# unirestore/UniRestore

Hardware: AMD Instinct MI355X
Metric: restored 512x512 images/sec @ 20 denoise steps (whole job) (higher is better)
Workload: dtype bf16; 1 GPU; PIR 512x512 batch=8/GPU, 20 DDIM steps, bf16, hipGraph replay (BASELINE.json configs[1]; configs[2] shape for N=8); global_batch=8, per_gpu_batch=8, image=512, denoise_steps=20, parallelism=image-parallel dp1, weights=seeded random init (no checkpoints reachable)

## Files before the change

### unirestore_amd/csrc/igemm.hip

```cpp
#include "igemm_impl.h"

namespace urk {
#define UR_DECLARE(name)                                                                                             \
  ConvLaunch name##_bf16(void* k, size_t ws_bytes);                                                                 \
  ConvLaunch name##_f16(void* k, size_t ws_bytes);                                                                  \
  static ConvLaunch name(ConvK& k, size_t ws_bytes) { return (k.f16 ? name##_f16 : name##_bf16)(&k, ws_bytes); }
UR_CONV_LAUNCHERS(UR_DECLARE)
#undef UR_DECLARE
}

namespace {

ConvLaunch dispatch_conv(ConvK& k, bool pair, size_t ws_bytes) {
  if (k.KH == 3 && k.stride == 1 && k.pad_t == 1 && k.pad_l == 1 && k.kcm && k.staged_ok_ && !pair && k.nbatch == 1 &&
      k.OW % 32 == 0 && k.OH % 8 == 0 && k.OH == (k.ups ? 2 * k.H : k.H) && k.OW == (k.ups ? 2 * k.W : k.W) && !k.yt) {
    const bool ok128 = k.Cout % 128 == 0, ok160 = k.Cout % 160 == 0;
    const long long tm8 = (long long)k.N * (k.OH / 8) * (k.OW / 32);
    auto eff = [](long long t) { return t <= 128 ? (double)(t * (256 / t)) / 256.0 : (double)t / (double)(((t + 255) / 256) * 256); };
    const bool use160 = ok160 && (!ok128 || eff(tm8 * (k.Cout / 160)) >= eff(tm8 * (k.Cout / 128)));
    const long long tiles8 = tm8 * (use160 ? k.Cout / 160 : k.Cout / 128);
    if ((ok128 || ok160) && tiles8 >= 64) {
      if (use160) return urk::halo_8x32_160(k, ws_bytes);
      return urk::halo_8x32_128(k, ws_bytes);
    }
  }
  if (k.KH == 3 && k.stride == 1 && k.pad_t == 1 && k.pad_l == 1 && k.kcm && !pair && k.nbatch == 1 && !k.ups && k.C2 == 0 &&
      k.Cout <= 32 && k.OW % 32 == 0 && k.OH % 8 == 0 && k.OH == k.H && k.OW == k.W && !k.yt && !k.gn_part && !k.gn_ab && !k.row_stats && !k.ln_stats &&
      !k.bias_img && (long long)k.N * (k.OH / 8) * (k.OW / 32) >= 128)
    return urk::halo_thin_32(k, ws_bytes);
  const bool himg_ups = k.ups && k.OH == 16 && k.OW == 16 && k.H == 8 && k.W == 8;
  if (k.KH == 3 && k.stride == 1 && k.pad_t == 1 && k.pad_l == 1 && k.kcm && k.staged_ok_ && !pair && k.nbatch == 1 &&
      ((!k.ups && k.OH == k.H && k.OW == k.W) || himg_ups) && !k.yt && k.Cout % 128 == 0 && k.nk >= 36) {
    if (k.wf && k.OH == 8 && k.OW == 8 && k.N <= 16 && k.Cin % 256 == 0 && k.nk >= 72 && k.y && k.ws && !k.gn_ab && !k.row_stats && !k.ln_stats &&
        (long long)(k.nk / 36) * k.M * k.Cout * 4 <= (long long)ws_bytes)
      return urk::wstream_8x8(k, ws_bytes);
    if (k.OH == 16 && k.OW == 16) return urk::himg_16x16(k, ws_bytes);
    if (k.OH == 8 && k.OW == 8 && k.N % 4 == 0) {
      return urk::himg_8x8x4(k, ws_bytes);
    }
  }
  if (k.KH == 1 && k.stride == 1 && !k.ups && k.C2 == 0 && k.staged_ok_ && k.Cout % 256 == 0 && !k.yt && (k.act == UR_ACT_GEGLU || k.act == UR_ACT_GATE) &&
      (long long)((k.M + 255) / 256) * (k.Cout / 256) * k.nbatch >= 200 && (long long)k.M * k.ldx < (1ll << 31) - 256)
  {
    auto fill = [](long long t) { return (double)t / (double)(((t + 255) / 256) * 256); };
    const long long tm = (k.M + 255) / 256;
    if (k.Cout % 320 == 0 && k.nbatch == 1 && !k.bias_img && fill(tm * (k.Cout / 320)) > fill(tm * (k.Cout / 256)))
      return urk::gemm_256x320_pair(k, ws_bytes);
    return urk::gemm_256x256(k, ws_bytes);
  }
  const bool use_v1 = k.KH == 1 && k.nk <= 10;
  const long long blocks128 = (long long)((k.M + 127) / 128) * ((k.Cout + 127) / 128) * k.nbatch;
  const bool g1 = k.KH == 1 && k.stride == 1 && !k.ups && k.C2 == 0 && k.pad_t == 0 && k.pad_l == 0 && k.OH == k.H && k.OW == k.W &&
                  (long long)k.M * k.ldx + k.Ktot < (1ll << 31) - 256;
  auto nosplit = [&](int bm, int bn) { return (long long)((k.M + bm - 1) / bm) * ((k.Cout + bn - 1) / bn) * k.nbatch >= 200 || k.nk < 8 || !k.ws; };
  if (k.KH == 1 && !pair && k.Cout > 64) {
    const long long blocks64 = (long long)((k.M + 63) / 64) * ((k.Cout + 63) / 64) * k.nbatch;
    if (blocks128 < 200 && g1 && blocks64 >= 128 && blocks64 <= 256 && k.nk >= 8 && k.nk <= 48) return urk::g1_64x64_deep(k, ws_bytes);
    if (g1 && blocks128 < 200 && k.nk > 24 && k.nk <= 96 && (long long)((k.M + 127) / 128) * ((k.Cout + 63) / 64) * k.nbatch >= 256)
      return urk::g1_128x64_deep(k, ws_bytes);
    if (blocks128 < 200 && g1 && ((blocks64 >= 128 && k.nk <= 24) || (blocks64 >= 256 && k.nk <= 48))) return urk::g1_64x64(k, ws_bytes);
    if (blocks128 < 200 && k.nk <= 24) return g1 && nosplit(64, 64) ? urk::g1_64x64(k, ws_bytes) : urk::v1_64x64(k, ws_bytes);
    if (use_v1 && blocks128 > 256 && blocks128 < 400 && k.Cout % 128 == 0) return g1 && nosplit(128, 64) ? urk::g1_128x64(k, ws_bytes) : urk::v1_128x64(k, ws_bytes);
  }
  if (use_v1) {
    if (pair) return urk::v1_128x128(k, ws_bytes);
    if (k.Cout <= 32) return urk::v1_256x32(k, ws_bytes);
    if (k.Cout <= 64) return urk::v1_128x64(k, ws_bytes);
    if (k.Cout % 160 == 0 && k.Cout % 128 != 0) return g1 && nosplit(128, 160) ? urk::g1_128x160(k, ws_bytes) : urk::v1_128x160(k, ws_bytes);
    return g1 && nosplit(128, 128) ? urk::g1_128x128(k, ws_bytes) : urk::v1_128x128(k, ws_bytes);
  }
  if (k.Cout <= 32) return urk::v2_256x32(k, ws_bytes);
  if (k.Cout <= 64 && !pair) return urk::v2_128x64(k, ws_bytes);
  const bool n160 = !pair && k.Cout % 160 == 0 && k.Cout % 128 != 0;
  const long long big_tiles = (long long)((k.M + 255) / 256) * ((k.Cout + (n160 ? 159 : 127)) / (n160 ? 160 : 128)) * k.nbatch;
  if (g1 && !pair && big_tiles < 256) {
    const long long t160 = k.Cout % 160 == 0 ? (long long)((k.M + 127) / 128) * (k.Cout / 160) : 0;
    const long long t128 = (long long)((k.M + 127) / 128) * ((k.Cout + 127) / 128);
    auto fill = [](long long t) { return t <= 0 ? 0.0 : (double)t / (double)(((t + 255) / 256) * 256); };
    if (t160 >= 200 && fill(t160) >= fill(t128)) return urk::g1_128x160(k, ws_bytes);
    if (t128 >= 200) return urk::g1_128x128(k, ws_bytes);
  }
  if (big_tiles >= 160) {
    if (n160 && g1) return urk::g1_128x160(k, ws_bytes);
    if (n160) return urk::v2_256x160(k, ws_bytes);
    return urk::v2_256x128(k, ws_bytes);
  }
  if (k.Cout % 160 == 0 && k.Cout % 128 != 0 && !pair) return urk::v1_128x160(k, ws_bytes);
  return urk::v1_128x128(k, ws_bytes);
}

}

static int conv_impl(const ur_conv_desc* d, ur_stream_t stream, ur_conv_plan* plan, ur_conv_launch_info* info = nullptr) {
  UR_REQUIRE(d && d->x && d->w, "null x/w");
  UR_REQUIRE(d->KH == d->KW && (d->KH == 1 || d->KH == 3), "only 1x1 and 3x3 kernels");
  UR_REQUIRE(d->C1 > 0 && d->C1 % 8 == 0 && d->C2 % 8 == 0 && d->ldx % 8 == 0, "Cin/ldx must be multiples of 8");
  UR_REQUIRE(d->C2 == 0 || (d->x2 && d->ldx2 % 8 == 0), "virtual concat needs x2");
  UR_REQUIRE(d->Cout > 0 && d->Cout % 4 == 0 && d->ldw % 8 == 0, "Cout%4, ldw%8");
  UR_REQUIRE(d->nbatch >= 1 && d->stride >= 1 && d->OH > 0 && d->OW > 0, "bad dims");
  UR_REQUIRE(d->y || d->yt || d->gn_part, "no output requested");
  UR_REQUIRE_DT(d->dtype);
  const bool pair = d->act == UR_ACT_GEGLU || d->act == UR_ACT_GATE;
  if (pair && d->Cout % 64 != 0)
    return ur::fail(UR_E_UNSUPPORTED, "ur_conv2d_nhwc: pair activations (GEGLU / SimpleGate) need Cout % 64 == 0 (32-row a|g interleave)");
  UR_REQUIRE(!d->y || (d->out_f32 ? d->ldy % 4 == 0 : d->ldy % 4 == 0), "ldy%4");
  UR_REQUIRE(!d->residual || d->ldr % 4 == 0, "ldr%4");
  UR_REQUIRE(!d->yt || (d->t_rows > 0 && d->n_split % 4 == 0 && !pair), "bad transposed-output spec");

  ConvK k;
  k.x = (const uint16_t*)d->x; k.x2 = (const uint16_t*)d->x2; k.w = (const uint16_t*)d->w; k.bias = d->bias;
  k.res = (const uint16_t*)d->residual; k.y = d->y; k.yt = (uint16_t*)d->yt;
  k.ws = d->workspace;
  k.N = d->N; k.H = d->H; k.W = d->W; k.C1 = d->C1; k.ldx = d->ldx; k.C2 = d->C2; k.ldx2 = d->ldx2;
  k.Cin = d->C1 + d->C2; k.Cout = d->Cout; k.ldw = d->ldw; k.ldy = d->ldy; k.ldr = d->ldr;
  k.KH = d->KH; k.KW = d->KW; k.stride = d->stride; k.pad_t = d->pad_t; k.pad_l = d->pad_l;
  k.OH = d->OH; k.OW = d->OW; k.OHW = d->OH * d->OW; k.ups = d->upsample2x; k.act = d->act; k.out_f32 = d->out_f32;
  k.n_split = d->yt ? d->n_split : d->Cout; k.t_rows = d->t_rows; k.t_ld = d->t_ld;
  k.out_scale = d->out_scale;
  k.M = d->N * d->OH * d->OW; k.Ktot = d->KH * d->KW * k.Cin; k.nk = (k.Ktot + 63) / 64; k.nbatch = d->nbatch;
  k.bs_x = d->bs_x; k.bs_x2 = d->bs_x2; k.bs_w = d->bs_w; k.bs_bias = d->bs_bias; k.bs_y = d->bs_y; k.bs_r = d->bs_r; k.bias_img = d->bias_img_stride;
  UR_REQUIRE(k.M > 0, "empty problem");
  UR_REQUIRE((long long)d->N * d->H * d->W * (long long)std::max(d->ldx, d->ldx2) < (1ll << 31) &&
                 (long long)d->Cout * d->ldw < (1ll << 31), "tensor too large for 32-bit element offsets");

  k.kcm = d->k_chunk_major; k.wf = (const uint16_t*)d->w_frag; k.wmajor = 0; k.xgm = 0; k.xbn = 0; k.patch_tw = 0;
  UR_REQUIRE(!k.kcm || (k.Cin % 64 == 0 && d->C1 % 64 == 0), "k_chunk_major needs C1 and C1+C2 to be multiples of 64");
  k.gn_part = d->gn_part; k.gn_ab = d->gn_ab; k.gn_silu = d->gn_silu; k.f16 = d->dtype == UR_DT_F16; k.gn_fused = 0; k.gn_parts = 0;
  k.ln_parts = d->ln_parts;
  k.row_stats = d->row_stats; k.ln_stats = d->ln_stats; k.ln_colsum = d->ln_colsum; k.ln_eps = d->ln_eps; k.ln_dim = d->ln_dim;
  UR_REQUIRE(!d->ln_stats || (d->ln_colsum && d->ln_dim > 0), "ln_stats needs ln_colsum / ln_dim");
  UR_REQUIRE(!(d->bias_img_stride && (pair || d->ln_stats || d->yt)), "per-image bias rows do not combine with pair activations / LayerNorm folding / transposed columns");
  k.staged_ok_ = (d->y ? (!d->out_f32 && ((d->ldy | d->bs_y) & 7) == 0) : d->gn_part != nullptr) &&
                 (!d->residual || ((d->ldr | d->bs_r) & 7) == 0);
  UR_REQUIRE(!d->gn_part || (!d->out_f32 && !d->yt), "gn_part needs a plain 16-bit output (or none)");
  hipStream_t s = (hipStream_t)stream;
  const double flops = 2.0 * k.M * (double)k.Cout * k.Ktot * k.nbatch;
  const double bytes = 2.0 * ((double)k.M * k.Cin + (double)k.Cout * k.Ktot + (double)k.M * k.Cout) * k.nbatch;
  const char* fam = d->KH == 3 ? "conv3x3_igemm" : "gemm1x1_igemm";
  static const bool prof_shapes = getenv("UR_PROF_SHAPES") != nullptr;
  if (prof_shapes) {
    static std::map<std::string, int> interned;
    char buf[128];
    snprintf(buf, sizeof buf, "%s M%d N%d K%d s%d u%d b%d a%d", d->KH == 3 ? "c3" : "g1", k.M, k.Cout, k.Ktot, d->stride, d->upsample2x,
             k.nbatch, d->act);
    fam = interned.emplace(buf, 0).first->first.c_str();
  }
  const ConvLaunch launch = dispatch_conv(k, pair, d->workspace_bytes);
  const bool group_loop = k.nbatch > 1 && d->KH == 3 && k.kcm && k.stride == 1 && !pair && !k.gn_part && !k.row_stats && !k.ln_stats &&
                          !k.yt && !k.gn_ab && !k.out_f32 && k.staged_ok_ && k.Cout % 128 == 0 && !k.bias_img && k.C2 == 0;
  auto group_k = [&](int b) {
    ConvK kb = k;
    kb.nbatch = 1;
    kb.x = k.x + b * k.bs_x; kb.w = k.w + b * k.bs_w; kb.bias = k.bias ? k.bias + b * k.bs_bias : nullptr;
    kb.res = k.res ? k.res + b * k.bs_r : nullptr;
    kb.y = reinterpret_cast<uint16_t*>(k.y) + b * k.bs_y;
    kb.bs_x = kb.bs_w = kb.bs_bias = kb.bs_y = kb.bs_r = 0;
    return kb;
  };
  if (plan) {
    plan->row_stat_parts = d->row_stats ? (k.splitk > 1 ? 1 : k.tiles_n) : 0;
    plan->gn_parts = k.gn_parts; plan->gn_fused = k.gn_fused; plan->prologue_ok = launch.prologue_ok;
  }
  if (info) {
    ConvK kb = group_loop ? group_k(0) : k;
    const ConvLaunch l = group_loop ? dispatch_conv(kb, pair, d->workspace_bytes) : launch;
    info->launcher = l.id; info->splitk = kb.splitk; info->nk_per_split = kb.nk_per_split;
    const ReducePlan r = kb.splitk > 1 ? plan_splitk_reduce(kb) : ReducePlan{-1, 0};
    info->reduce = r.kind; info->reduce_ri = r.ri;
    info->gn_pass = k.gn_part && !k.gn_fused && !group_loop;
    info->group_loop = group_loop;
  }
  if (plan || info) return UR_OK;
  if (!d->y && d->gn_part && (!k.gn_fused || k.splitk > 1))
    return ur::fail(UR_E_UNSUPPORTED, "ur_conv2d_nhwc: y == NULL needs a launch whose epilogue writes gn_part (see ur_conv2d_plan)");
// ... 70 lines not shown
```

### unirestore_amd/csrc/igemm_impl.h

```cpp
#pragma once
#include <cstdio>
#include <cstdlib>
#include <map>
#include <string>

#include "common.h"

static __device__ uint4 g_zero_page[8];
typedef uint32_t ig_u32x4 __attribute__((ext_vector_type(4)));

struct ConvLaunch {
  int (*launch)(void* k, hipStream_t s);
  int prologue_ok;
  int id;
};

namespace {

struct ConvK {
  const uint16_t* x; const uint16_t* x2; const uint16_t* w; const float* bias; const uint16_t* res;
  void* y; uint16_t* yt; float* ws; float* gn_part; const float* gn_ab;
  float* row_stats; const float* ln_stats; const float* ln_colsum; float ln_eps; int ln_dim, ln_parts;
  int N, H, W, C1, ldx, C2, ldx2, Cin, Cout, ldw, ldy, ldr, KH, KW, stride, pad_t, pad_l, OH, OW, OHW;
  int ups, act, out_f32, n_split, t_rows, t_ld;
// ... 1594 lines not shown
    unsigned wvo[WPIECES];
#pragma unroll
    for (int q = 0; q < WPIECES; ++q) {
      const int row = n0 + q * 8 + lr;
      wvo[q] = row < p.Cout ? (unsigned)row * (unsigned)p.ldw * 2u + ((q & 1) ? ck1 : ck0) : IG_OOB;
    }
    int hpx[HNEED];
    auto dma_w = [&](int kt, int ring, int q0, int q1) {
      const unsigned so = (unsigned)(kt0 + min(kt, nk - 1)) * 128u;
#pragma unroll
      for (int q = q0; q < q1; ++q) ig_lds_dma16(wring_lds + ring * WBYTES + q * 1024, wvo[q], rs_w, so);
    };
    auto dma_h = [&](int c, int h) {
      const int cb = (c_begin + min(c, nchunk - 1)) * 64;
      const bool second = cb >= p.C1;
      const unsigned ld2 = (unsigned)(second ? p.ldx2 : p.ldx) * 2u;
      const unsigned so = (unsigned)(second ? cb - p.C1 : cb) * 2u;
#pragma unroll
      for (int j = 0; j < HPER; ++j) {
        const int q = h * HPER + j;
        if (h < 16 && q < HNEED) {
          const unsigned vo = hpx[q] >= 0 ? (unsigned)hpx[q] * ld2 + ((q & 1) ? ck1 : ck0) : IG_OOB;
          const unsigned m0v = hbuf_lds + (c & 1) * HBYTES + q * 1024;
          if (second) ig_lds_dma16(m0v, vo, rs_x2, so);
          else ig_lds_dma16(m0v, vo, rs_x1, so);
        }
      }
    };
    auto halo_count = [](int h) -> int { return (h >= 16 || h * HPER >= HNEED) ? 0 : (HNEED - h * HPER < HPER ? HNEED - h * HPER : HPER); };
    auto dma_ab = [&](int c) {
      const unsigned vo = lane < 32 ? (unsigned)((img * 2 + (lane >> 4 & 1)) * p.Cin + (lane & 15) * 4) * 4u : IG_OOB;
      ig_lds_dma16(abuf_lds + (c & 1) * 1024, vo, rs_ab, (unsigned)((c_begin + min(c, nchunk - 1)) * 64) * 4u);
    };
    if (gnp && do_h) dma_ab(0);
    if (do_w) dma_w(1, 1, 0, WPIECES);
    if (do_h) {
#pragma unroll
      for (int q = 0; q < HNEED; ++q) hpx[q] = halo_pixel(q * 8 + lr);
    }
    if (gnp && do_h) {
      if (do_w) asm volatile("s_waitcnt vmcnt(%0)" ::"n"(WPIECES) : "memory");
      else asm volatile("s_waitcnt vmcnt(0)" ::: "memory");
    }
    __builtin_amdgcn_s_barrier();
    if (gnp) __builtin_amdgcn_s_barrier();
    for (int c = 0; c < nchunk; ++c) {
#pragma unroll
      for (int tap = 0; tap < 9; ++tap) {
        const int kt = c * 9 + tap;
        if (do_w) dma_w(kt + 2, (tap + 2) % 3, 0, WH);
        if (do_h) {
          dma_h(c + 1, 2 * tap);
          if (gnp && tap == 0) dma_ab(c + 1);
        }
        if (kt + 1 == nk) asm volatile("s_waitcnt vmcnt(0)" ::: "memory");
        else if (do_w && do_h) asm volatile("s_waitcnt vmcnt(%0)" ::"n"(WH + halo_count(2 * tap) + ((gnp && tap == 0) ? 1 : 0)) : "memory");
        else if (do_w) asm volatile("s_waitcnt vmcnt(%0)" ::"n"(WH) : "memory");
        else asm volatile("s_waitcnt vmcnt(%0)" ::"n"(halo_count(2 * tap) + ((gnp && tap == 0) ? 1 : 0)) : "memory");
        __builtin_amdgcn_s_barrier();
        if (kt + 1 < nk) {
          if (do_w) dma_w(kt + 2, (tap + 2) % 3, WH, WPIECES);
          if (do_h) dma_h(c + 1, 2 * tap + 1);
        }
        __builtin_amdgcn_s_barrier();
      }
    }
    return;
  }

  const int wm = wid % WM, wn = wid / WM;
  const int chunk = ps ^ ((((wid & 1) << 2) + (lr >> 1)) & 7);
  static_assert(HTAP % 2 == 0, "piece parity");
  int hpix[8];
#pragma unroll
  for (int t = 0; t < 8; ++t) hpix[t] = (wid < HTAP && t * HTAP + wid < HNEED) ? halo_pixel((t * HTAP + wid) * 8 + lr) : -1;
  {
    const ig_u32x4 rs_w = ig_make_rsrc(p.w, (unsigned long long)p.Cout * p.ldw * 2);
    const int cb = c_begin * 64;
    const bool second = cb >= p.C1;
    const ig_u32x4 rs_x = second ? ig_make_rsrc(p.x2, (unsigned long long)p.N * p.H * p.W * p.ldx2 * 2) : ig_make_rsrc(p.x, (unsigned long long)p.N * p.H * p.W * p.ldx * 2);
    const unsigned ld2 = (unsigned)(second ? p.ldx2 : p.ldx) * 2u, so = (unsigned)(second ? cb - p.C1 : cb) * 2u;
    if (wid_s < HTAP) {
#pragma unroll
      for (int t = 0; t < 8; ++t)
        if (t * HTAP + wid_s < HNEED)
          ig_lds_dma16(hbuf_lds + (t * HTAP + wid_s) * 1024, hpix[t] >= 0 ? (unsigned)hpix[t] * ld2 + chunk * 16u : IG_OOB, rs_x, so);
    }
#pragma unroll
    for (int j = 0; j < (WPIECES + NW - 1) / NW; ++j) {
      const int q = wid_s + NW * j;
      if (q < WPIECES) {
        const int row = n0 + q * 8 + lr;
        ig_lds_dma16(wring_lds + q * 1024, row < p.Cout ? (unsigned)row * (unsigned)p.ldw * 2u + chunk * 16u : IG_OOB, rs_w, (unsigned)kt0 * 128u);
      }
    }
  }
  auto gn_slot = [&](int c, int t) {
    if (hpix[t] >= 0)
      gn_piece_inplace<F16>(hbuf + (c & 1) * HBYTES + (t * HTAP + wid) * 1024 + lane * 16, gn_load_ab(abuf + (c & 1) * 1024, chunk), p.gn_silu != 0);
  };
  f32x16 acc[FN][FM];
#pragma unroll
  for (int a = 0; a < FN; ++a)
#pragma unroll
    for (int b = 0; b < FM; ++b)
#pragma unroll
      for (int e = 0; e < 16; ++e) acc[a][b][e] = 0.f;
  const int frow = lane & 31, fhalf = lane >> 5;
  const unsigned aw_lds = wring_lds + (wn * WTN + frow) * 128 + ((fhalf ^ ((frow >> 1) & 7)) << 4);
  static_assert(((WTN >> 1) & 7) == 0, "the wave's weight rows must keep the swizzle phase of fragment row 0");
  auto tap_addr = [&](int cc, int tp, unsigned (&ab)[FM]) -> unsigned {
    const int dy = tp / 3, dx = tp % 3;
#pragma unroll
    for (int b = 0; b < FM; ++b) {
      const int hrow = (wm * FM + b + dy) * PW + dx + frow;
      ab[b] = hbuf_lds + (cc & 1) * HBYTES + hrow * 128 + ((fhalf ^ ((hrow >> 1) & 7)) << 4);
    }
    return aw_lds + (tp % 3) * WBYTES;
  };
  KPipeRings<FM, FN> rings;
  kpipe_init(rings);
  asm volatile("s_waitcnt vmcnt(0)" ::: "memory");
  __builtin_amdgcn_s_barrier();
  if (gnp) {
#pragma unroll
    for (int t = 0; t < 8; ++t) gn_slot(0, t);
    asm volatile("s_waitcnt lgkmcnt(0)" ::: "memory");
    __builtin_amdgcn_s_barrier();
  }
  {
    unsigned ab0[FM];
    const unsigned aw0 = tap_addr(0, 0, ab0);
    kpipe<FM, FN, F16, 0>(acc, rings, ab0, aw0, ab0, aw0);
  }
  for (int c = 0; c < nchunk; ++c) {
    const bool next_chunk = c + 1 < nchunk;
#pragma unroll
    for (int tap = 0; tap < 9; ++tap) {
      if (gnp && tap >= 2 && next_chunk) gn_slot(c + 1, tap >= 2 ? tap - 2 : 0);
      if (gnp && tap == 0 && c > 0) gn_slot(c, 7);
      unsigned ab[FM], abn[FM];
      const unsigned aw = tap_addr(c, tap, ab), awn = tap_addr(c + (tap == 8 ? 1 : 0), (tap + 1) % 9, abn);
      kpipe<FM, FN, F16, 1>(acc, rings, ab, aw, abn, awn);
      __builtin_amdgcn_s_barrier();
      kpipe<FM, FN, F16, 2>(acc, rings, ab, aw, abn, awn);
      __builtin_amdgcn_s_barrier();
    }
  }
  kpipe_drain(rings);
  asm volatile("s_nop 15\n\ts_nop 7" ::: "memory");
  igemm_epilogue<FM, FN, WTM, WTN, BM, BN, NT, F16, false>(p, acc, m0, n0, wm, wn, lane, 0, sz, smem);
}

template <int TH, int BN, int WM, int WN>
struct HaloThin {
  static constexpr int NW = WM * WN, HPIX = (TH + 2) * 34, HSLOTS = (HPIX + 8 * NW - 1) / (8 * NW);
  static constexpr int HBYTES = HSLOTS * NW * 1024;
  static constexpr int lds = 2 * HBYTES + 3 * (BN * 128 > NW * 1024 ? BN * 128 : NW * 1024) + 2048;
  static_assert(lds <= 160 * 1024, "LDS budget");
  static int plan(ConvK& k, size_t) {
    k.tiles_m = k.N * (k.OH / TH) * (k.OW / 32);
    k.tiles_n = (k.Cout + BN - 1) / BN;
    k.splitk = 1;
    k.nk_per_split = k.nk;
    set_gn_plan(k, false, 0);
    return 0;
  }
  static int launch(ConvK& k, hipStream_t s) {
    k.patch_tw = 32;
    static ur::DeviceOnce attr_once;
    if (auto once_guard = attr_once.first()) {
      hipFuncSetAttribute(reinterpret_cast<const void*>(&igemm_halo_kernel<TH, BN, WM, WN, UR_TU_F16 != 0, false>), hipFuncAttributeMaxDynamicSharedMemorySize, lds);
    }
    UR_F16_SWITCH(k, hipLaunchKernelGGL((igemm_halo_kernel<TH, BN, WM, WN, F16, false>), dim3(k.tiles_m * k.tiles_n, 1), dim3(NW * 64), lds, s, k));
    return ur::check_launch("ur_conv2d_nhwc");
  }
};

template <int TH, int BN, int WM, int WN>
struct Halo {
  static constexpr int NW = WM * WN, BM = TH * 32, HPIX = (TH + 2) * 34, HSLOTS = (HPIX + 8 * NW - 1) / (8 * NW);
  static constexpr int HBYTES = HSLOTS * NW * 1024;
  static constexpr int lds_loop = 2 * HBYTES + 3 * BN * 128 + 2048, lds_epi = epi_lds_bytes<BM, BN, NW * 64>();
  static constexpr int lds = lds_loop > lds_epi ? lds_loop : lds_epi;
  static_assert(lds <= 160 * 1024, "LDS budget");
  static constexpr bool GN_OK = BN <= 128;
  static int plan(ConvK& k, size_t ws_bytes) {
    k.tiles_m = k.N * (k.OH / TH) * (k.OW / 32);
    k.tiles_n = (k.Cout + BN - 1) / BN;
    const int nchunk = k.nk / 9;
    const long long tiles = (long long)k.tiles_m * k.tiles_n;
    plan_splitk(k, ws_bytes, tiles <= 128 && k.ws && k.y ? std::min<long long>(256 / tiles, std::max(1, nchunk / 2)) : 1, 9);
    set_gn_plan(k, true, (k.OH / TH) * (k.OW / 32));
    return GN_OK;
  }
  static int launch(ConvK& k, hipStream_t s) {
    k.patch_tw = 32;
    static ur::DeviceOnce attr_once;
    if (auto once_guard = attr_once.first()) {
      hipFuncSetAttribute(reinterpret_cast<const void*>(&igemm_halo_kernel<TH, BN, WM, WN, UR_TU_F16 != 0, false>), hipFuncAttributeMaxDynamicSharedMemorySize, lds);
      hipFuncSetAttribute(reinterpret_cast<const void*>(&igemm_halo_kernel<TH, BN, WM, WN, UR_TU_F16 != 0, GN_OK>), hipFuncAttributeMaxDynamicSharedMemorySize, lds);
      hipFuncSetAttribute(reinterpret_cast<const void*>(&igemm_halo_ws_kernel<TH, BN, WM, WN, UR_TU_F16 != 0, false>), hipFuncAttributeMaxDynamicSharedMemorySize, lds);
      hipFuncSetAttribute(reinterpret_cast<const void*>(&igemm_halo_ws_kernel<TH, BN, WM, WN, UR_TU_F16 != 0, GN_OK>), hipFuncAttributeMaxDynamicSharedMemorySize, lds);
    }
    static const bool no_ws = getenv("UR_HALO_NOWS") != nullptr;
    if (no_ws) {
      if (GN_OK && k.gn_ab) UR_F16_SWITCH(k, hipLaunchKernelGGL((igemm_halo_kernel<TH, BN, WM, WN, F16, GN_OK>), dim3(k.tiles_m * k.tiles_n, k.splitk), dim3(NW * 64), lds, s, k));
      else UR_F16_SWITCH(k, hipLaunchKernelGGL((igemm_halo_kernel<TH, BN, WM, WN, F16, false>), dim3(k.tiles_m * k.tiles_n, k.splitk), dim3(NW * 64), lds, s, k));
    } else {
      static const bool ld1 = getenv("UR_HALO_LD1") != nullptr;
      const dim3 blk((NW + (ld1 ? 1 : 2)) * 64);
      if (GN_OK && k.gn_ab) UR_F16_SWITCH(k, hipLaunchKernelGGL((igemm_halo_ws_kernel<TH, BN, WM, WN, F16, GN_OK>), dim3(k.tiles_m * k.tiles_n, k.splitk), blk, lds, s, k));
      else UR_F16_SWITCH(k, hipLaunchKernelGGL((igemm_halo_ws_kernel<TH, BN, WM, WN, F16, false>), dim3(k.tiles_m * k.tiles_n, k.splitk), blk, lds, s, k));
    }
    if (k.splitk > 1) {
      k.patch_tw = 0;
      launch_splitk_reduce(k, s);
    }
    return ur::check_launch("ur_conv2d_nhwc");
  }
};

template <int TH, int TW, int NIMG, int BN, int WM, int WN, bool F16, bool GNP>
__global__ __launch_bounds__(WM* WN * 64) void igemm_halo_img_kernel(const ConvK p) {
  constexpr int NW = WM * WN, BM = TH * TW * NIMG, PW = TW + 2, HP = (TH + 2) * PW, HPIX = HP * NIMG;
  constexpr int HSLOTS = (HPIX + 8 * NW - 1) / (8 * NW);
  constexpr int HPIECES = HSLOTS * NW, HBYTES = HPIECES * 1024;
  constexpr int WBYTES = BN * 128, WPIECES = BN / 8, WPW = (WPIECES + NW - 1) / NW;
  constexpr int WTM = BM / WM, WTN = BN / WN, FM = WTM / 32, FN = WTN / 32, NT = NW * 64;
  static_assert(BM == 256 && NW == 8 && WTM % 32 == 0 && WTN % 32 == 0 && HSLOTS <= 8, "tile shape");
  extern __shared__ __attribute__((aligned(16))) unsigned char smem[];
  unsigned char* const hbuf = smem;
  unsigned char* const wring = smem + 2 * HBYTES;
  unsigned char* const abuf = wring + 3 * WBYTES;
  constexpr bool GN_OK = NIMG == 1 && HSLOTS <= 7;
  constexpr bool gnp = GN_OK && GNP;

  const int tid = threadIdx.x, lane = tid & 63, wid = tid >> 6;
  const int wm = wid % WM, wn = wid / WM;
  int sz = blockIdx.y, tn, tmi;
  if (p.wmajor) {
    const int L = blockIdx.x, xcd = L & 7, j = L >> 3;
    const int g = (j / p.tiles_m) * 8 + xcd;
    if (g >= p.tiles_n * p.splitk) return;
    tn = g % p.tiles_n; sz = g / p.tiles_n; tmi = j % p.tiles_m;
  } else {
    int id = blockIdx.x;
    const int nt = p.tiles_m * p.tiles_n, q = nt >> 3, r = nt & 7, xcd = id & 7, idx = id >> 3;
    id = (xcd < r ? xcd * (q + 1) : r * (q + 1) + (xcd - r) * q) + idx;
    tn = id % p.tiles_n; tmi = id / p.tiles_n;
  }
  const int n0 = tn * BN, img0 = tmi * NIMG, m0 = tmi * BM;

  typedef __attribute__((address_space(1))) const void* gptr_t;
  typedef __attribute__((address_space(3))) void* lptr_t;
  const uint16_t* __restrict__ X1 = p.x;
  const uint16_t* __restrict__ X2 = p.x2;
  const uint16_t* __restrict__ Wt = p.w;
  const uint16_t* zero = reinterpret_cast<const uint16_t*>(g_zero_page);
  const int lr = lane >> 3, ps = lane & 7;

  int hpix[HSLOTS], hchk[HSLOTS];
#pragma unroll
  for (int t = 0; t < HSLOTS; ++t) {
    const int hr = (t * NW + wid) * 8 + lr;
    const int im = hr / HP, rin = hr - im * HP, hy = rin / PW, hx = rin - hy * PW;
    const int iy = hy - 1, ix = hx - 1;
    const bool v = hr < HPIX && img0 + im < p.N && (unsigned)iy < (unsigned)TH && (unsigned)ix < (unsigned)TW;
    const int sy = p.ups ? iy >> 1 : iy, sx = p.ups ? ix >> 1 : ix;
    hpix[t] = v ? ((img0 + im) * p.H + sy) * p.W + sx : -1;
    hchk[t] = ps ^ (((rin >> 1) - hy) & 7);
  }
  const int wchunk = ps ^ ((((wid & 1) << 2) + (lr >> 1)) & 7);
  int woff[WPW];
#pragma unroll
  for (int i = 0; i < WPW; ++i) {
    const int qq = (wid + NW * i < WPIECES) ? wid + NW * i : wid;
    const int row = n0 + qq * 8 + lr;
    woff[i] = row < p.Cout ? row * p.ldw : -1;
  }
  const int nchunk_all = p.nk / 9, cps = p.nk_per_split / 9;
  const int c_begin = sz * cps, c_end = min(nchunk_all, c_begin + cps);
  const int nchunk = c_end - c_begin, nk = nchunk * 9, kt0 = c_begin * 9;

  const int wid_s = __builtin_amdgcn_readfirstlane(wid);
  const ig_u32x4 rs_w = ig_make_rsrc(Wt, (unsigned long long)p.Cout * p.ldw * 2);
  const ig_u32x4 rs_x1 = ig_make_rsrc(X1, (unsigned long long)p.N * p.H * p.W * p.ldx * 2);
  const ig_u32x4 rs_x2 = ig_make_rsrc(X2 ? X2 : X1, (unsigned long long)p.N * p.H * p.W * (X2 ? p.ldx2 : p.ldx) * 2);
  const unsigned wring_lds = (unsigned)(uintptr_t)(lptr_t)wring, hbuf_lds = (unsigned)(uintptr_t)(lptr_t)hbuf;
  unsigned wvo[WPW];
#pragma unroll
  for (int i = 0; i < WPW; ++i) wvo[i] = woff[i] >= 0 ? (unsigned)woff[i] * 2u + wchunk * 16u : IG_OOB;
  auto issue_w = [&](int kt, int ring) {
#pragma unroll
    for (int i = 0; i < WPW; ++i) {
      const int qq = (wid_s + NW * i < WPIECES) ? wid_s + NW * i : wid_s;
      ig_lds_dma16(wring_lds + ring * WBYTES + qq * 1024, wvo[i], rs_w, (unsigned)(kt0 + kt) * 128u);
    }
  };
  auto issue_h = [&](int c, int t) {
    const int cb = (c_begin + c) * 64;
    const bool second = cb >= p.C1;
    const unsigned ld2 = (unsigned)(second ? p.ldx2 : p.ldx) * 2u;
    const unsigned vo = hpix[t] >= 0 ? (unsigned)hpix[t] * ld2 + hchk[t] * 16u : IG_OOB;
    const unsigned m0v = hbuf_lds + (c & 1) * HBYTES + (t * NW + wid_s) * 1024;
    if (second) ig_lds_dma16(m0v, vo, rs_x2, (unsigned)(cb - p.C1) * 2u);
    else ig_lds_dma16(m0v, vo, rs_x1, (unsigned)cb * 2u);
  };
  auto issue_ab = [&](int c) {
    const float* t = p.gn_ab + ((long long)img0 * 2 + (lane >> 4 & 1)) * p.Cin + (c_begin + c) * 64 + (lane & 15) * 4;
    const void* g = lane < 32 ? (const void*)t : (const void*)zero;
    __builtin_amdgcn_global_load_lds((gptr_t)g, (lptr_t)(abuf + (c & 1) * 1024), 16, 0, 0);
  };
  auto gn_slot = [&](int c, int t) {
    if (hpix[t] >= 0)
      gn_piece_inplace<F16>(hbuf + (c & 1) * HBYTES + (t * NW + wid) * 1024 + lane * 16, gn_load_ab(abuf + (c & 1) * 1024, hchk[t]), p.gn_silu != 0);
  };

  f32x16 acc[FN][FM];
#pragma unroll
  for (int a = 0; a < FN; ++a)
#pragma unroll
    for (int b = 0; b < FM; ++b)
#pragma unroll
      for (int e = 0; e < 16; ++e) acc[a][b][e] = 0.f;
  const int frow = lane & 31, fhalf = lane >> 5;
  int hrow0[FM], hin0[FM], hy0[FM];
#pragma unroll
  for (int b = 0; b < FM; ++b) {
    const int pix = wm * WTM + b * 32 + frow;
    const int im = pix / (TH * TW), r = pix - im * (TH * TW), y = r / TW, x = r - y * TW;
    hin0[b] = y * PW + x;
    hrow0[b] = im * HP + hin0[b];
    hy0[b] = y;
  }
  const unsigned hb_lds = (unsigned)(uintptr_t)(lptr_t)hbuf;
  const unsigned aw_lds = (unsigned)(uintptr_t)(lptr_t)wring + (wn * WTN + frow) * 128 + ((fhalf ^ ((frow >> 1) & 7)) << 4);
  static_assert(((WTN >> 1) & 7) == 0, "the wave's weight rows must keep the swizzle phase of fragment row 0");

  if (gnp) issue_ab(0);
#pragma unroll
  for (int t = 0; t < HSLOTS; ++t) issue_h(0, t);
  issue_w(0, 0);
  if (nk > 1) {
    issue_w(1, 1);
    asm volatile("s_waitcnt vmcnt(%0)" ::"n"(WPW) : "memory");
  } else {
    asm volatile("s_waitcnt vmcnt(0)" ::: "memory");
  }
  if (gnp) {
#pragma unroll
    for (int t = 0; t < HSLOTS; ++t) gn_slot(0, t);
    asm volatile("s_waitcnt lgkmcnt(0)" ::: "memory");
  }
  __builtin_amdgcn_s_barrier();

  for (int c = 0; c < nchunk; ++c) {
    const unsigned char* hb = hbuf + (c & 1) * HBYTES;
    const bool next_chunk = c + 1 < nchunk;
// ... 259 lines not shown
```

Before: 30.14 images/s.

## Add warp-specialized halo implicit-GEMM kernel for stride-2 3x3 convolutions

Adds a halo-tiled implicit-GEMM kernel for stride-2 3x3 convolutions. It splits the input patch into four parity planes (even/odd rows and columns) and walks the nine taps grouped by plane. Two loader waves stream the weight ring and the parity-plane patches with counted vmcnt waits, so loads overlap the MFMA waves. Dispatch sends large stride-2 downsampling convs (more than 128 tiles, Cin >= 256) to this kernel instead of the generic path, and stride-2 disables the GroupNorm-fused plan. This adds complex hand-scheduled synchronisation, which is a correctness risk for padding and odd shapes.

```diff
diff --git a/unirestore_amd/csrc/igemm.hip b/unirestore_amd/csrc/igemm.hip
--- a/unirestore_amd/csrc/igemm.hip
+++ b/unirestore_amd/csrc/igemm.hip
@@ -12,14 +12,15 @@
 namespace {
 
 ConvLaunch dispatch_conv(ConvK& k, bool pair, size_t ws_bytes) {
-  if (k.KH == 3 && k.stride == 1 && k.pad_t == 1 && k.pad_l == 1 && k.kcm && k.staged_ok_ && !pair && k.nbatch == 1 &&
-      k.OW % 32 == 0 && k.OH % 8 == 0 && k.OH == (k.ups ? 2 * k.H : k.H) && k.OW == (k.ups ? 2 * k.W : k.W) && !k.yt) {
+  const bool halo_s2 = k.stride == 2 && !k.ups && k.C2 == 0 && k.pad_t == k.pad_l && (k.pad_t == 0 || k.pad_t == 1) && k.H == 2 * k.OH && k.W == 2 * k.OW;
+  const bool halo_s1 = k.stride == 1 && k.pad_t == 1 && k.pad_l == 1 && k.OH == (k.ups ? 2 * k.H : k.H) && k.OW == (k.ups ? 2 * k.W : k.W);
+  if (k.KH == 3 && (halo_s1 || halo_s2) && k.kcm && k.staged_ok_ && !pair && k.nbatch == 1 && k.OW % 32 == 0 && k.OH % 8 == 0 && !k.yt) {
     const bool ok128 = k.Cout % 128 == 0, ok160 = k.Cout % 160 == 0;
     const long long tm8 = (long long)k.N * (k.OH / 8) * (k.OW / 32);
     auto eff = [](long long t) { return t <= 128 ? (double)(t * (256 / t)) / 256.0 : (double)t / (double)(((t + 255) / 256) * 256); };
     const bool use160 = ok160 && (!ok128 || eff(tm8 * (k.Cout / 160)) >= eff(tm8 * (k.Cout / 128)));
     const long long tiles8 = tm8 * (use160 ? k.Cout / 160 : k.Cout / 128);
-    if ((ok128 || ok160) && tiles8 >= 64) {
+    if ((ok128 || ok160) && (halo_s2 ? tiles8 > 128 && k.Cin >= 256 : tiles8 >= 64)) {
       if (use160) return urk::halo_8x32_160(k, ws_bytes);
       return urk::halo_8x32_128(k, ws_bytes);
     }
diff --git a/unirestore_amd/csrc/igemm_impl.h b/unirestore_amd/csrc/igemm_impl.h
--- a/unirestore_amd/csrc/igemm_impl.h
+++ b/unirestore_amd/csrc/igemm_impl.h
@@ -1770,6 +1770,196 @@
   igemm_epilogue<FM, FN, WTM, WTN, BM, BN, NT, F16, false>(p, acc, m0, n0, wm, wn, lane, 0, sz, smem);
 }
 
+struct S2Walk {
+  static constexpr int tap_of(int pos) { return pos == 0 ? 0 : pos == 1 ? 2 : pos == 2 ? 6 : pos == 3 ? 8 : pos == 4 ? 1 : pos == 5 ? 7 : pos == 6 ? 4 : pos == 7 ? 3 : 5; }
+  static constexpr int group_of(int pos) { return pos < 4 ? 0 : pos < 6 ? 1 : pos < 7 ? 2 : 3; }
+  static constexpr int dy_even(int g) { return g < 2; }
+  static constexpr int dx_even(int g) { return g == 0 || g == 3; }
+  static constexpr int cols(int g) { return 32 + dx_even(g); }
+  static constexpr int pieces(int th, int g) { return ((th + dy_even(g)) * cols(g) + 7) / 8; }
+  static constexpr int base(int th, int g) { return g == 0 ? 0 : base(th, g - 1) + pieces(th, g - 1); }
+  static constexpr int sched_group(int h) { return h < 6 ? 1 : (h == 8 || h == 9) ? 2 : h == 12 ? 3 : (h == 14 || h == 15) ? 0 : -1; }
+  static constexpr int sched_per(int th, int h) {
+    return h < 6 ? (pieces(th, 1) + 5) / 6 : (h == 8 || h == 9) ? (pieces(th, 2) + 1) / 2 : h == 12 ? pieces(th, 3) : (pieces(th, 0) + 1) / 2;
+  }
+  static constexpr int sched_first(int th, int h) { return h < 6 ? h * sched_per(th, h) : (h == 9 || h == 15) ? sched_per(th, h) : 0; }
+  static constexpr int sched_count(int th, int h) {
+    const int g = sched_group(h);
+    if (g < 0) return 0;
+    const int left = pieces(th, g) - sched_first(th, h);
+    return left < 0 ? 0 : left < sched_per(th, h) ? left : sched_per(th, h);
+  }
+};
+template <int TH, int BN, int WM, int WN, bool F16>
+__global__ __launch_bounds__((WM * WN + 2) * 64) void igemm_halo_s2_kernel(const ConvK p) {
+  constexpr int NW = WM * WN, TW = 32, BM = TH * TW;
+  constexpr int HNEED = S2Walk::pieces(TH, 0), HBYTES = HNEED * 1024;
+  constexpr int NPIECE = S2Walk::base(TH, 3) + S2Walk::pieces(TH, 3), MAXG = S2Walk::pieces(TH, 3);
+  constexpr int HPER = (HNEED + 15) / 16, HTAP = 2 * HPER;
+  constexpr int WBYTES = BN * 128, WPIECES = BN / 8, WH = WPIECES / 2;
+  constexpr int WTM = BM / WM, WTN = BN / WN, FM = WTM / 32, FN = WTN / 32, NT = NW * 64;
+  static_assert(NW == 8 && WTM % 32 == 0 && WTN % 32 == 0 && HTAP <= NW && 8 * HTAP >= HNEED && ktile_asm_ok<FM, FN>(), "wave layout");
+  static_assert(S2Walk::pieces(TH, 1) <= HNEED && S2Walk::pieces(TH, 2) <= HNEED && S2Walk::pieces(TH, 3) <= HNEED, "patch buffers");
+  extern __shared__ __attribute__((aligned(16))) unsigned char smem[];
+  unsigned char* const hbuf = smem;
+  unsigned char* const wring = smem + 2 * HBYTES;
+  unsigned* const tbl = reinterpret_cast<unsigned*>(wring + 3 * WBYTES);
+  typedef __attribute__((address_space(3))) void* lptr_t;
+
+  const int tid = threadIdx.x, lane = tid & 63, wid = tid >> 6;
+  const int wid_s = __builtin_amdgcn_readfirstlane(wid);
+  const int sz = blockIdx.y;
+  int id = blockIdx.x;
+  {
+    const int nt = p.tiles_m * p.tiles_n, q = nt >> 3, r = nt & 7, xcd = id & 7, idx = id >> 3;
+    id = (xcd < r ? xcd * (q + 1) : r * (q + 1) + (xcd - r) * q) + idx;
+  }
+  const int tn = id % p.tiles_n, tmi = id / p.tiles_n;
+  const int tiles_x = p.OW / TW, tiles_y = p.OH / TH;
+  const int tx = tmi % tiles_x, ty = (tmi / tiles_x) % tiles_y, img = tmi / (tiles_x * tiles_y);
+  const int n0 = tn * BN;
+  const int m0 = img * p.OHW + ty * TH * p.OW + tx * TW;
+  const int cps = p.nk_per_split / 9, c_begin = sz * cps, nchunk = min(p.nk / 9, c_begin + cps) - c_begin;
+  const int kt0 = c_begin * 9;
+  const unsigned wring_lds = (unsigned)(uintptr_t)(lptr_t)wring, hbuf_lds = (unsigned)(uintptr_t)(lptr_t)hbuf;
+  const int lr = lane >> 3, ps = lane & 7;
+  const unsigned ld2 = (unsigned)p.ldx * 2u;
+  auto plane_offset = [&](int g, int hr) -> unsigned {
+    const int de = S2Walk::dy_even(g), xe = S2Walk::dx_even(g), pw = 32 + xe;
+    const int hy = hr / pw, hx = hr - hy * pw;
+    const int iy = 2 * (ty * TH + hy - (de & p.pad_t)) + ((de ^ 1) ^ p.pad_t);
+    const int ix = 2 * (tx * TW + hx - (xe & p.pad_l)) + ((xe ^ 1) ^ p.pad_l);
+    const bool v = hy < TH + de && (unsigned)iy < (unsigned)p.H && (unsigned)ix < (unsigned)p.W;
+    return v ? (unsigned)((img * p.H + iy) * p.W + ix) * ld2 : IG_OOB;
+  };
+
+  if (wid_s >= NW) {
+    const bool do_w = wid_s == NW;
+    const unsigned ck0 = (ps ^ ((lr >> 1) & 7)) * 16u, ck1 = (ps ^ ((4 + (lr >> 1)) & 7)) * 16u;
+    const ig_u32x4 rs_w = ig_make_rsrc(p.w, (unsigned long long)p.Cout * p.ldw * 2);
+    const ig_u32x4 rs_x = ig_make_rsrc(p.x, (unsigned long long)p.N * p.H * p.W * p.ldx * 2);
+    unsigned wvo[WPIECES];
+#pragma unroll
+    for (int q = 0; q < WPIECES; ++q) {
+      const int row = n0 + q * 8 + lr;
+      wvo[q] = row < p.Cout ? (unsigned)row * (unsigned)p.ldw * 2u + ((q & 1) ? ck1 : ck0) : IG_OOB;
+    }
+    auto dma_w = [&](int c, int pos, int ring, int q0, int q1) {
+      const unsigned so = (unsigned)(kt0 + min(c, nchunk - 1) * 9 + S2Walk::tap_of(pos)) * 128u;
+#pragma unroll
+      for (int q = q0; q < q1; ++q) ig_lds_dma16(wring_lds + ring * WBYTES + q * 1024, wvo[q], rs_w, so);
+    };
+    auto dma_h = [&](int c, int h) {
+      const int g = S2Walk::sched_group(h), first = S2Walk::sched_first(TH, h), cnt = S2Walk::sched_count(TH, h);
+      if (g < 0) return;
+      const unsigned so = (unsigned)(c_begin + (g == 0 ? min(c + 1, nchunk - 1) : c)) * 128u;
+      const unsigned* t = tbl + (S2Walk::base(TH, g) + first) * 8 + lr;
+#pragma unroll
+      for (int j = 0; j < MAXG; ++j)
+        if (j < cnt)
+          ig_lds_dma16(hbuf_lds + (g & 1) * HBYTES + (first + j) * 1024, t[j * 8] + (((first + j) & 1) ? ck1 : ck0), rs_x, so);
+    };
+    if (do_w) dma_w(0, 1, 1, 0, WPIECES);
+    else {
+      for (int i = lane; i < NPIECE * 8; i += 64) {
+        const int q = i >> 3;
+        const int g = q < S2Walk::base(TH, 1) ? 0 : q < S2Walk::base(TH, 2) ? 1 : q < S2Walk::base(TH, 3) ? 2 : 3;
+        const int b = g == 0 ? 0 : g == 1 ? S2Walk::base(TH, 1) : g == 2 ? S2Walk::base(TH, 2) : S2Walk::base(TH, 3);
+        tbl[i] = plane_offset(g, (q - b) * 8 + (i & 7));
+      }
+    }
+    __builtin_amdgcn_s_barrier();
+    constexpr int H0 = S2Walk::sched_count(TH, 0), H8 = S2Walk::sched_count(TH, 8), H14 = S2Walk::sched_count(TH, 14);
+    static_assert(S2Walk::sched_count(TH, 2) == H0 && S2Walk::sched_count(TH, 4) == H0 && S2Walk::sched_count(TH, 6) == 0 &&
+                  S2Walk::sched_count(TH, 10) == 0 && S2Walk::sched_count(TH, 16) == 0 && H14 < 64, "counted vmcnt of the patch loader");
+    for (int c = 0; c < nchunk; ++c) {
+#pragma unroll
+      for (int pos = 0; pos < 9; ++pos) {
+        const bool last = c + 1 == nchunk && pos == 8;
+        if (do_w) dma_w(c + (pos + 2) / 9, (pos + 2) % 9, (pos + 2) % 3, 0, WH);
+        else dma_h(c, 2 * pos);
+        if (last || (!do_w && pos == 6)) asm volatile("s_waitcnt vmcnt(0)" ::: "memory");
+        else if (do_w) asm volatile("s_waitcnt vmcnt(%0)" ::"n"(WH) : "memory");
+        else if (pos < 3) asm volatile("s_waitcnt vmcnt(%0)" ::"n"(H0) : "memory");
+        else if (pos == 4) asm volatile("s_waitcnt vmcnt(%0)" ::"n"(H8) : "memory");
+        else if (pos == 7) asm volatile("s_waitcnt vmcnt(%0)" ::"n"(H14) : "memory");
+        else asm volatile("s_waitcnt vmcnt(0)" ::: "memory");
+        __builtin_amdgcn_s_barrier();
+        if (!last) {
+          if (do_w) dma_w(c + (pos + 2) / 9, (pos + 2) % 9, (pos + 2) % 3, WH, WPIECES);
+          else dma_h(c, 2 * pos + 1);
+        }
+        __builtin_amdgcn_s_barrier();
+      }
+    }
+    return;
+  }
+
+  const int wm = wid % WM, wn = wid / WM;
+  const int chunk = ps ^ ((((wid & 1) << 2) + (lr >> 1)) & 7);
+  static_assert(HTAP % 2 == 0, "piece parity");
+  {
+    const ig_u32x4 rs_w = ig_make_rsrc(p.w, (unsigned long long)p.Cout * p.ldw * 2);
+    const ig_u32x4 rs_x = ig_make_rsrc(p.x, (unsigned long long)p.N * p.H * p.W * p.ldx * 2);
+    if (wid_s < HTAP) {
+#pragma unroll
+      for (int t = 0; t < 8; ++t)
+        if (t * HTAP + wid_s < HNEED)
+          ig_lds_dma16(hbuf_lds + (t * HTAP + wid_s) * 1024, plane_offset(0, (t * HTAP + wid) * 8 + lr) + chunk * 16u, rs_x, (unsigned)c_begin * 128u);
+    }
+#pragma unroll
+    for (int j = 0; j < (WPIECES + NW - 1) / NW; ++j) {
+      const int q = wid_s + NW * j;
+      if (q < WPIECES) {
+        const int row = n0 + q * 8 + lr;
+        ig_lds_dma16(wring_lds + q * 1024, row < p.Cout ? (unsigned)row * (unsigned)p.ldw * 2u + chunk * 16u : IG_OOB, rs_w, (unsigned)kt0 * 128u);
+      }
+    }
+  }
+  f32x16 acc[FN][FM];
+#pragma unroll
+  for (int a = 0; a < FN; ++a)
+#pragma unroll
+    for (int b = 0; b < FM; ++b)
+#pragma unroll
+      for (int e = 0; e < 16; ++e) acc[a][b][e] = 0.f;
+  const int frow = lane & 31, fhalf = lane >> 5;
+  const unsigned aw_lds = wring_lds + (wn * WTN + frow) * 128 + ((fhalf ^ ((frow >> 1) & 7)) << 4);
+  static_assert(((WTN >> 1) & 7) == 0, "the wave's weight rows must keep the swizzle phase of fragment row 0");
+  auto tap_addr = [&](int pos, unsigned (&ab)[FM]) -> unsigned {
+    const int g = S2Walk::group_of(pos), tp = S2Walk::tap_of(pos), ry = (tp / 3) >> 1, rx = (tp % 3) >> 1;
+#pragma unroll
+    for (int b = 0; b < FM; ++b) {
+      const int hrow = (wm * FM + b + ry) * S2Walk::cols(g) + rx + frow;
+      ab[b] = hbuf_lds + (g & 1) * HBYTES + hrow * 128 + ((fhalf ^ ((hrow >> 1) & 7)) << 4);
+    }
+    return aw_lds + (pos % 3) * WBYTES;
+  };
+  KPipeRings<FM, FN> rings;
+  kpipe_init(rings);
+  asm volatile("s_waitcnt vmcnt(0)" ::: "memory");
+  __builtin_amdgcn_s_barrier();
+  {
+    unsigned ab0[FM];
+    const unsigned aw0 = tap_addr(0, ab0);
+    kpipe<FM, FN, F16, 0>(acc, rings, ab0, aw0, ab0, aw0);
+  }
+  for (int c = 0; c < nchunk; ++c) {
+#pragma unroll
+    for (int pos = 0; pos < 9; ++pos) {
+      unsigned ab[FM], abn[FM];
+      const unsigned aw = tap_addr(pos, ab), awn = tap_addr((pos + 1) % 9, abn);
+      kpipe<FM, FN, F16, 1>(acc, rings, ab, aw, abn, awn);
+      __builtin_amdgcn_s_barrier();
+      kpipe<FM, FN, F16, 2>(acc, rings, ab, aw, abn, awn);
+      __builtin_amdgcn_s_barrier();
+    }
+  }
+  kpipe_drain(rings);
+  asm volatile("s_nop 15\n\ts_nop 7" ::: "memory");
+  igemm_epilogue<FM, FN, WTM, WTN, BM, BN, NT, F16, false>(p, acc, m0, n0, wm, wn, lane, 0, sz, smem);
+}
+
 template <int TH, int BN, int WM, int WN>
 struct HaloThin {
   static constexpr int NW = WM * WN, HPIX = (TH + 2) * 34, HSLOTS = (HPIX + 8 * NW - 1) / (8 * NW);
@@ -1802,6 +1992,9 @@
   static constexpr int lds_loop = 2 * HBYTES + 3 * BN * 128 + 2048, lds_epi = epi_lds_bytes<BM, BN, NW * 64>();
   static constexpr int lds = lds_loop > lds_epi ? lds_loop : lds_epi;
   static_assert(lds <= 160 * 1024, "LDS budget");
+  static constexpr int lds_loop_s2 = 2 * S2Walk::pieces(TH, 0) * 1024 + 3 * BN * 128 + (S2Walk::base(TH, 3) + S2Walk::pieces(TH, 3)) * 32;
+  static constexpr int lds_s2 = lds_loop_s2 > lds_epi ? lds_loop_s2 : lds_epi;
+  static_assert(lds_s2 <= 160 * 1024, "LDS budget");
   static constexpr bool GN_OK = BN <= 128;
   static int plan(ConvK& k, size_t ws_bytes) {
     k.tiles_m = k.N * (k.OH / TH) * (k.OW / 32);
@@ -1810,7 +2003,7 @@
     const long long tiles = (long long)k.tiles_m * k.tiles_n;
     plan_splitk(k, ws_bytes, tiles <= 128 && k.ws && k.y ? std::min<long long>(256 / tiles, std::max(1, nchunk / 2)) : 1, 9);
     set_gn_plan(k, true, (k.OH / TH) * (k.OW / 32));
-    return GN_OK;
+    return GN_OK && k.stride == 1;
   }
   static int launch(ConvK& k, hipStream_t s) {
     k.patch_tw = 32;
@@ -1820,9 +2013,12 @@
       hipFuncSetAttribute(reinterpret_cast<const void*>(&igemm_halo_kernel<TH, BN, WM, WN, UR_TU_F16 != 0, GN_OK>), hipFuncAttributeMaxDynamicSharedMemorySize, lds);
       hipFuncSetAttribute(reinterpret_cast<const void*>(&igemm_halo_ws_kernel<TH, BN, WM, WN, UR_TU_F16 != 0, false>), hipFuncAttributeMaxDynamicSharedMemorySize, lds);
       hipFuncSetAttribute(reinterpret_cast<const void*>(&igemm_halo_ws_kernel<TH, BN, WM, WN, UR_TU_F16 != 0, GN_OK>), hipFuncAttributeMaxDynamicSharedMemorySize, lds);
+      hipFuncSetAttribute(reinterpret_cast<const void*>(&igemm_halo_s2_kernel<TH, BN, WM, WN, UR_TU_F16 != 0>), hipFuncAttributeMaxDynamicSharedMemorySize, lds_s2);
     }
     static const bool no_ws = getenv("UR_HALO_NOWS") != nullptr;
-    if (no_ws) {
+    if (k.stride == 2) {
+      UR_F16_SWITCH(k, hipLaunchKernelGGL((igemm_halo_s2_kernel<TH, BN, WM, WN, F16>), dim3(k.tiles_m * k.tiles_n, k.splitk), dim3((NW + 2) * 64), lds_s2, s, k));
+    } else if (no_ws) {
       if (GN_OK && k.gn_ab) UR_F16_SWITCH(k, hipLaunchKernelGGL((igemm_halo_kernel<TH, BN, WM, WN, F16, GN_OK>), dim3(k.tiles_m * k.tiles_n, k.splitk), dim3(NW * 64), lds, s, k));
       else UR_F16_SWITCH(k, hipLaunchKernelGGL((igemm_halo_kernel<TH, BN, WM, WN, F16, false>), dim3(k.tiles_m * k.tiles_n, k.splitk), dim3(NW * 64), lds, s, k));
     } else {
```

Result: no change. 30.12 images/s (-0.1%).
